# jacklishufan/InstructAny2Pix

Hardware: AMD Instinct MI355X
Metric: denoise-steps/sec (512x512, 50-step DDIM, batch 8) (higher is better)
Workload: dtype f16; 1 GPU; BASELINE configs[2]: 512x512, latent [8,4,64,64], 50-step DDIM, ctx 81 (77 text + 4 IP tokens), SDXL-base UNet + IP-Adapter; global_batch=8, parallelism=dp1, context_kv=projected in every step (reference schedule, as rounds 1-4), ranks=1, dist_backend=none (single process), weight_broadcast_route=none

## Files before the change

### instructany2pix_amd/csrc/attention_core.h

```cpp
#pragma once
#include "common.h"

#define MASKED (-1.0e30f)
#ifndef IA2P_ATTN_DMA
#define IA2P_ATTN_DMA 1
#endif
#ifndef IA2P_ATTN_PK
#define IA2P_ATTN_PK 1
#endif

__device__ __forceinline__ fp16x4 lds_tr16(const char* p) {
  return __builtin_amdgcn_ds_read_tr16_b64_v4f16((fp16x4 __attribute__((address_space(3)))*)p);
}

template <int NT>
__device__ __forceinline__ void stage_kv(const half_t* Kb, const half_t* Vb, int ld, int s0, int nsk, int tid, char* sK, char* sV) {
  typedef unsigned int u4 __attribute__((ext_vector_type(4)));
  u4 kreg[2 * NT], vreg[2 * NT];
#pragma unroll
  for (int u = 0; u < 2 * NT; ++u) {
    const int c = tid + 256 * u, row = c >> 3, pos = c & 7;
    const size_t off = (size_t)(s0 + min(row, nsk - 1)) * ld + pos * 8;
    kreg[u] = *(const u4*)(Kb + off);
    vreg[u] = *(const u4*)(Vb + off);
// ... 38 lines not shown
    if (write) {
      *(u4*)(sK + lrow * 128 + ((pos ^ ((lrow >> 1) & 7)) << 4)) = kreg[u] & keep;
      *(u4*)(sV + lrow * 128 + ((pos ^ (((lrow >> 1) & 1) << 2)) << 4)) = vreg[u] & keep;
    }
  }
}

typedef unsigned int attn_u4 __attribute__((ext_vector_type(4)));
constexpr int ATTN_PRE_TILES = 3;
struct AttnKvRegs { attn_u4 k[2 * ATTN_PRE_TILES], v[2 * ATTN_PRE_TILES]; };
__device__ __host__ __forceinline__ bool attn_kv_resident(const AttnArgs& p) {
  return ((p.seg[0].nkeys + 63) >> 6) + (p.nseg == 2 ? (p.seg[1].nkeys + 63) >> 6 : 0) <= ATTN_PRE_TILES;
}
__device__ __forceinline__ void attn_kv_load(const AttnArgs& p, int b, int hd, int tid, AttnKvRegs& rg) {
  typedef unsigned int u4 __attribute__((ext_vector_type(4)));
  const int nt0 = (p.seg[0].nkeys + 63) >> 6;
  const bool two = p.nseg == 2;
  const AttnSeg sg1 = two ? p.seg[1] : p.seg[0];
  const half_t* K0 = p.seg[0].K + (size_t)b * p.seg[0].rows_per_batch * p.seg[0].ld + hd * 64;
  const half_t* V0 = p.seg[0].V + (size_t)b * p.seg[0].rows_per_batch * p.seg[0].ld + hd * 64;
  const half_t* K1 = sg1.K + (size_t)b * sg1.rows_per_batch * sg1.ld + hd * 64;
  const half_t* V1 = sg1.V + (size_t)b * sg1.rows_per_batch * sg1.ld + hd * 64;
#pragma unroll
  for (int u = 0; u < 2 * ATTN_PRE_TILES; ++u) {
    const bool s1 = (u >> 1) >= nt0;
    const int c = tid + 256 * u, row = (c >> 3) - (s1 ? nt0 * 64 : 0), pos = c & 7;
    const size_t off = (size_t)min(row, (s1 ? sg1.nkeys : p.seg[0].nkeys) - 1) * (s1 ? sg1.ld : p.seg[0].ld) + pos * 8;
    rg.k[u] = *(const u4*)((s1 ? K1 : K0) + off);
    rg.v[u] = *(const u4*)((s1 ? V1 : V0) + off);
  }
}
template <bool FOLD = false>
__device__ __forceinline__ void attn_kv_store(const AttnArgs& p, int tid, const AttnKvRegs& rg, char* sK, char* sV) {
  typedef unsigned int u4 __attribute__((ext_vector_type(4)));
  const int n0 = p.seg[0].nkeys, n1 = p.nseg == 2 ? p.seg[1].nkeys : 0;
  const int nt0 = (n0 + 63) >> 6, nt = nt0 + ((n1 + 63) >> 6);
  const bool fold = FOLD && !(p.xcd_map & 4) && n1 > 0 && attn_fold_ok(n0, n1);
#pragma unroll
  for (int u = 0; u < 2 * ATTN_PRE_TILES; ++u) {
    if ((u >> 1) >= nt || (fold && u > 2 * nt0)) break;
    const bool s1 = (u >> 1) >= nt0;
    const int c = tid + 256 * u, pos = c & 7;
    int lrow = c >> 3;
    const int row = lrow - (s1 ? nt0 * 64 : 0);
    const unsigned keep = row < (s1 ? n1 : n0) ? 0xFFFFFFFFu : 0u;
    bool write = true;
    if (fold) {
      if (s1) { write = row < n1; lrow = n0 + row; }
      else write = lrow < n0 || lrow >= n0 + n1;
    }
    if (write) {
      *(u4*)(sK + lrow * 128 + ((pos ^ ((lrow >> 1) & 7)) << 4)) = rg.k[u] & keep;
      *(u4*)(sV + lrow * 128 + ((pos ^ (((lrow >> 1) & 1) << 2)) << 4)) = rg.v[u] & keep;
    }
  }
}

template <int MODE, bool PRE = false>
__device__ __forceinline__ void attn_core(const AttnArgs& p, int b, int hd, const h8 (&qf)[4], char* sK, char* sV, int tid, f16v (&otot)[2]) {
  const int lane = tid & 63;
  const int r31 = lane & 31, hh = lane >> 5;
  (void)r31;
  f16v o[2];
  float mrun = MASKED, lrun = 0.f;
#pragma unroll
  for (int d = 0; d < 2; ++d)
#pragma unroll
    for (int r = 0; r < 16; ++r) { o[d][r] = 0.f; if (MODE == 2) otot[d][r] = 0.f; }

  const int nt0 = (p.seg[0].nkeys + 63) >> 6, nt1 = p.nseg == 2 ? (p.seg[1].nkeys + 63) >> 6 : 0;
  const bool resident = PRE || (MODE != 0 && nt0 + nt1 <= 4);
  const int n0 = p.seg[0].nkeys, n1 = p.nseg == 2 ? p.seg[1].nkeys : 0;
  const bool fold = MODE == 1 && resident && !(p.xcd_map & 4) && attn_fold_ok(n0, n1);
  if (resident && !PRE) {
    const half_t* K0 = p.seg[0].K + (size_t)b * p.seg[0].rows_per_batch * p.seg[0].ld + hd * 64;
    const half_t* V0 = p.seg[0].V + (size_t)b * p.seg[0].rows_per_batch * p.seg[0].ld + hd * 64;
    const half_t* K1 = p.seg[1].K + (size_t)b * p.seg[1].rows_per_batch * p.seg[1].ld + hd * 64;
    const half_t* V1 = p.seg[1].V + (size_t)b * p.seg[1].rows_per_batch * p.seg[1].ld + hd * 64;
    switch (nt0 + nt1) {
      case 2: stage_kv2<2>(K0, V0, p.seg[0].ld, p.seg[0].nkeys, K1, V1, p.seg[1].ld, p.seg[1].nkeys, nt0, tid, sK, sV, fold); break;
      case 3: stage_kv2<3>(K0, V0, p.seg[0].ld, p.seg[0].nkeys, K1, V1, p.seg[1].ld, p.seg[1].nkeys, nt0, tid, sK, sV, fold); break;
      default: stage_kv2<4>(K0, V0, p.seg[0].ld, p.seg[0].nkeys, K1, V1, p.seg[1].ld, p.seg[1].nkeys, nt0, tid, sK, sV, fold); break;
    }
    __syncthreads();
  }
  float lt = 1.f;
  constexpr int NSEG = MODE == 0 ? 1 : 2;
#pragma unroll 1
  for (int sg = 0; sg < NSEG; ++sg) {
    if (MODE == 1 && fold && sg == 1) break;
    AttnSeg seg = sg == 0 ? p.seg[0] : p.seg[1];
    if (sg == 1 && p.w1_b) seg.weight = p.w1_b[b];
    const half_t* Kb = seg.K + (size_t)b * seg.rows_per_batch * seg.ld + hd * 64;
    const half_t* Vb = seg.V + (size_t)b * seg.rows_per_batch * seg.ld + hd * 64;
    const bool ip_tile = MODE == 1 && sg == 1;
    if (MODE == 2 || ip_tile) { mrun = MASKED; lrun = 0.f; }
    if (MODE == 2) {
#pragma unroll
      for (int d = 0; d < 2; ++d)
#pragma unroll
        for (int r = 0; r < 16; ++r) o[d][r] = 0.f;
    }

    constexpr bool DMA = IA2P_ATTN_DMA && MODE == 0 && !PRE;
    constexpr int SSZ = DMA ? 128 : 256;
    auto stage_dma = [&](int s0n, int buf) {
// ... 267 lines not shown
```

### instructany2pix_amd/csrc/gemm_epilogue.h

```cpp
#pragma once
#include "gemm_tile.h"
#include "gn_fold.h"

template <int BM, int BN, int NSTAGE, int WGM, int BK, int PP, int WGN, int XA, int HALO>
__device__ __forceinline__ void tile_epilogue(f4 (&acc)[BM / WGM / 16][BN / WGN / 16], const TileCtx& tc, const GemmArgs& p, const AttnArgs* xa, AttnKvRegs& kvr) {
  constexpr int NWAVE = WGM * WGN;
  constexpr int WM = BM / WGM, WN = BN / WGN;
  constexpr int MR = WM / 16, NR = WN / 16;
  constexpr int MRH = MR / 2;
  extern __shared__ __attribute__((aligned(1024))) char smem[];
  const int tid = threadIdx.x;
  const int lane = tid & 63;
  const int wave = __builtin_amdgcn_readfirstlane(tid >> 6);
  const int hM = tc.hM, hN = tc.hN, hK = tc.hK, tm = tc.tm, tn = tc.tn, bm0 = tc.bm0, bn0 = tc.bn0, tiles_m = tc.tiles_m, tiles_n = tc.tiles_n, split = tc.split, nsplit = tc.nsplit;
  const float ln_s1 = tc.ln_s1, ln_s2 = tc.ln_s2;
  (void)tiles_m; (void)hK;
  auto row_m = [&](int r) { return HALO ? tc.h_m0 + (r >> 4) * p.Wo + (r & 15) : bm0 + r; };
  auto frag_row = [](int i) constexpr { return PP == 2 ? (i / (MR / 2)) * (BM / 2) + (i % (MR / 2)) * 16 : i * 16; };
  auto frag_col = [](int j) constexpr { return PP == 2 ? (j / (NR / 2)) * (BN / 2) + (j % (NR / 2)) * 16 : j * 16; };
  const int wm0 = (wave / WGN) * (PP == 2 ? WM / 2 : WM), wn0 = (wave % WGN) * (PP == 2 ? WN / 2 : WN);
  const int frow = lane & 15, fq = lane >> 4;
  using EC = EpiCfg<BM, BN, NSTAGE, WGM, BK, WGN, PP>;
  constexpr int PITCH = EC::PITCH;
  constexpr int NT = NWAVE * 64, CR = EC::CR;
  float* tile = (float*)smem;
  const bool reg_epi = XA == 0 && EC::REG_EPI && nsplit == 1 && p.vec8 != 0 && (hN & 7) == 0 && !p.act;
  char* cbase = smem + (reg_epi ? EC::T16_BYTES : EC::TILE_BYTES);
  float* ln_rows = (float*)cbase;
  float* ln_cs = ln_rows + 2 * BM;
  float* ln_lb = ln_cs + BN;
  int* sk_flag = (int*)(ln_lb + BN);
  float2* part = (float2*)(ln_lb + BN + 4);
  const float2* phi = (const float2*)(cbase + (reg_epi ? EC::EXTRA16 - EC::LUT_BYTES : EC::extra_nolut(CR)));
  __syncthreads();
  if (p.ln_stats) {
    if (tid < BM) {
      const float2 mr = ln_mean_rstd_f(ln_s1, ln_s2, hK, p.ln_eps);
      ln_rows[tid] = mr.x;
      ln_rows[BM + tid] = mr.y;
    }
    if constexpr (XA == 4) {
      if (tid < BN / 4) {
        const int n = ((tid * 4) >> 6) * (hN / 3) + tn * 64 + ((tid * 4) & 63);
        *(f4*)(ln_cs + tid * 4) = *(const f4*)(p.ln_cs + n);
        *(f4*)(ln_lb + tid * 4) = *(const f4*)(p.ln_bias + n);
      }
    } else if (tid < BN / 4 && bn0 + tid * 4 < hN) {
      *(f4*)(ln_cs + tid * 4) = *(const f4*)(p.ln_cs + bn0 + tid * 4);
      *(f4*)(ln_lb + tid * 4) = *(const f4*)(p.ln_bias + bn0 + tid * 4);
    }
  }
  unsigned pfacc = 0, pfv[8] = {0, 0, 0, 0, 0, 0, 0, 0};
  if ((PP == 1 || PP == 2) && p.pf) {
    const long nwg = (long)tiles_m * tiles_n * nsplit;
    const long per = ((p.pf_bytes + nwg - 1) / nwg + 255) & ~255L;
    const long lo = (long)blockIdx.x * per, hi = min(lo + per, p.pf_bytes & ~15L);
    const char* src = (const char*)p.pf;
    constexpr long SW = NWAVE * 64 * 16;
    if (lo < hi)
      for (long o = lo + tid * 16; o < hi; o += 8 * SW) {
#pragma unroll
        for (int u = 0; u < 8; ++u) pfacc ^= pfv[u];
#pragma unroll
        for (int u = 0; u < 8; ++u) pfv[u] = *(const unsigned*)(src + min(o + u * SW, hi - 16));
#ifdef IA2P_PP_EAGER_PF
#pragma unroll
        for (int u = 0; u < 8; ++u) asm volatile("" : "+v"(pfv[u]));
#endif
      }
  }
  auto pf_sink = [&]() {
    if (PP == 1 || PP == 2) asm volatile("" ::"v"(pfacc), "v"(pfv[0]), "v"(pfv[1]), "v"(pfv[2]), "v"(pfv[3]), "v"(pfv[4]), "v"(pfv[5]), "v"(pfv[6]), "v"(pfv[7]));
  };
  const float e_as = p.acc_scale == 0.f ? 1.f : p.acc_scale, e_bs = p.bias_scale == 0.f ? 1.f : p.bias_scale;
  const bool fast = p.vec8 != 0 && (hN & 7) == 0;
  const __amdgpu_buffer_rsrc_t c_rsrc = wt_rsrc((void*)p.C, (size_t)hM * p.ldc * 2);
  auto store_c8 = [&](size_t elem, h8 o) {
    if (p.c_wt) store16_wt(c_rsrc, elem * 2, o);
    else *(h8*)(p.C + elem) = o;
  };
  auto tl = [&](int r, int c) -> f4 { return *(const f4*)(tile + (size_t)r * PITCH + ((c ^ (r & 7)) << 2)); };
  auto acc_to_tile = [&](int ch) {
    if constexpr (PP == 2) {
      static_assert(PP != 2 || (EC::NCHUNK == 2 && CR == BM / 2), "8-phase tile: one epilogue chunk per row half");
      auto half = [&](auto h_tag) {
        constexpr int H = decltype(h_tag)::value;
// ... 20 lines not shown
        }
      }
    }
  };
  if constexpr (XA == 4) {
    static_assert(XA != 4 || (BM == 256 && BN == 192 && WGM == 4 && WGN == 2 && (PP == 0 || PP == 3)), "fused QKV + self-attention: 256 x 192 tiles, 8 waves");
    char* sK = smem;
    char* sV = smem + 32768;
    char* sQ = smem + 65536;
    __syncthreads();
#pragma unroll
    for (int i = 0; i < MR; ++i) {
      const int r = wm0 + i * 16 + frow;
      const float mu = p.ln_stats ? ln_rows[r] : 0.f, rs = p.ln_stats ? ln_rows[BM + r] : 1.f;
#pragma unroll
      for (int j = 0; j < NR; ++j) {
        const int cl = wn0 + j * 16 + fq * 4;
        float v[4] = {acc[i][j][0], acc[i][j][1], acc[i][j][2], acc[i][j][3]};
        if (p.ln_stats) {
#pragma unroll
          for (int e = 0; e < 4; ++e) v[e] = ln_fold_f(v[e], mu, rs, ln_cs[cl + e], ln_lb[cl + e]);
        } else if (p.bias) {
          const h4 hb = *(const h4*)(p.bias + (cl >> 6) * (hN / 3) + tn * 64 + (cl & 63));
#pragma unroll
          for (int e = 0; e < 4; ++e) v[e] += (float)hb[e];
        }
        h4 o;
#pragma unroll
        for (int e = 0; e < 4; ++e) o[e] = (half_t)v[e];
        const int which = cl >> 6, d = cl & 63, chunk = d >> 3, sub = (d & 7) * 2;
        const int sw = which == 0 ? (r & 7) : which == 1 ? ((r >> 1) & 7) : (((r >> 1) & 1) << 2);
        char* img = which == 0 ? sQ : which == 1 ? sK : sV;
        *(h4*)(img + r * 128 + ((chunk ^ sw) << 4) + sub) = o;
      }
    }
    __syncthreads();
    IA2P_STAMP(if (tid == 0 && p.partial) ((unsigned long long*)p.partial)[8 * blockIdx.x + 7] = __builtin_amdgcn_s_memrealtime();)
    const int r31 = lane & 31, hh = lane >> 5;
    h8 qf[4];
    {
      const int r = wave * 32 + r31;
#pragma unroll
      for (int s = 0; s < 4; ++s) qf[s] = *(const h8*)(sQ + r * 128 + (((2 * s + hh) ^ (r & 7)) << 4));
    }
    const AttnArgs& ap = *xa;
    f16v otot[2];
    attn_core<0, true>(ap, tm, tn, qf, sK, sV, tid, otot);
    IA2P_STAMP(if (tid == 0 && p.partial) ((unsigned long long*)p.partial)[8 * blockIdx.x + 6] = __builtin_amdgcn_s_memrealtime();)
    attn_store_o(otot, ap.O, (size_t)ap.B * ap.Nq * ap.ldo, tm, wave * 32, tn, ap.Nq, ap.ldo, sQ + wave * 4096, lane, (ap.xcd_map & 2) != 0);
    IA2P_STAMP(
      asm volatile("s_waitcnt vmcnt(0)" ::: "memory");
      __syncthreads();
      if (tid == 0 && p.partial) ((unsigned long long*)p.partial)[8 * blockIdx.x + 5] = __builtin_amdgcn_s_memrealtime();
    )
    return;
  } else if constexpr (XA != 0) {
    static_assert(BM == 128 && BN == 64 && WGM == 2 && WGN == 2 && !PP && EC::NCHUNK == 1, "fused cross-attention: 128 x 64 tiles, 4 waves");
    IA2P_STAMP(unsigned long long* xo = p.partial ? (unsigned long long*)p.partial + 8 * blockIdx.x : nullptr;)
    acc_to_tile(0);
    __syncthreads();
    const int r31 = lane & 31, hh = lane >> 5;
    h8 qf[4];
    {
      const int r = wave * 32 + r31;
      const float mu = p.ln_stats ? ln_rows[r] : 0.f, rs = p.ln_stats ? ln_rows[BM + r] : 1.f;
#pragma unroll
      for (int s = 0; s < 4; ++s) {
        const int cl = 16 * s + 8 * hh;
        const f4 x0 = tl(r, cl >> 2), x1 = tl(r, (cl >> 2) + 1);
        float v[8] = {x0[0], x0[1], x0[2], x0[3], x1[0], x1[1], x1[2], x1[3]};
        if (p.ln_stats) {
#pragma unroll
          for (int e = 0; e < 8; ++e) v[e] = ln_fold_f(v[e], mu, rs, ln_cs[cl + e], ln_lb[cl + e]);
        } else {
#pragma unroll
          for (int e = 0; e < 8; ++e) v[e] *= e_as;
          if (p.bias) {
            const h8 hb = *(const h8*)(p.bias + bn0 + cl);
#pragma unroll
            for (int e = 0; e < 8; ++e) v[e] = fmaf((float)hb[e], e_bs, v[e]);
          }
        }
#pragma unroll
        for (int e = 0; e < 8; ++e) qf[s][e] = (half_t)v[e];
      }
    }
    __syncthreads();
    const AttnArgs& ap = *xa;
    const int b = bm0 / ap.Nq, q0 = bm0 - b * ap.Nq + wave * 32, hd = tn;
    f16v otot[2];
    attn_kv_store<XA - 1 == 1>(ap, tid, kvr, smem, smem + 32768);
    __syncthreads();
    IA2P_STAMP(if (tid == 0 && xo) xo[6] = __builtin_amdgcn_s_memrealtime();)
    attn_core<XA - 1, true>(ap, b, hd, qf, smem, smem + 32768, tid, otot);
    __syncthreads();
    IA2P_STAMP(if (tid == 0 && xo) xo[7] = __builtin_amdgcn_s_memrealtime();)
    attn_store_o(otot, ap.O, (size_t)ap.B * ap.Nq * ap.ldo, b, q0, hd, ap.Nq, ap.ldo, smem + wave * 4096, lane, (ap.xcd_map & 2) != 0);
  IA2P_STAMP(
    asm volatile("s_waitcnt vmcnt(0)" ::: "memory");
    __syncthreads();
    if (tid == 0 && xo) xo[5] = __builtin_amdgcn_s_memrealtime();
  )
    return;
  }
  if constexpr (XA == 0 && EC::REG_EPI) {
  if (reg_epi) {
// ... 542 lines not shown
```

### instructany2pix_amd/csrc/gemm_kernel.h

```cpp
#pragma once
#include "gemm_epilogue.h"

template <int BM, int BN, int NSTAGE, bool CONV, int WGM = 2, int BK = 64, int PP = 0, int WGN = 2, int XA = 0, bool SUB = false>
__device__ __forceinline__ void gemm_tile_body(const half_t* hA, const half_t* hW, const half_t* hzero, int hM, int hN, int hK, int hlda, int hldw, int hrpb, int hbstride,
                                               int hroff, int hsplitk, int hgroup_w, int hflags, const GemmArgs& p, const AttnArgs* xa, const float* pre_ln_stats = nullptr, int pre_ln_slots = 0, int bid0 = 0) {
  static_assert(PP != 1 || (WGM * WGN == 8 && (WGM == 4 || WGM == 8) && NSTAGE == 3), "ping-pong schedule: 8 waves (two groups of 4 by tile rows), 3-stage ring");
  static_assert(PP != 3 || (WGM == 4 && NSTAGE == 2 && !CONV), "two-slot ping-pong schedule: 8 waves, 2 k-tile slots");
  static_assert(PP != 2 || (WGM == 2 && WGN == 4 && NSTAGE == 2 && BK == 64 && BM == 256 && (BN == 256 || BN == 128) && XA == 0), "8-phase schedule: 256-row tiles, 2 x 4 waves, two k-tile buffers");
  constexpr int NWAVE = WGM * WGN;
  constexpr int WM = BM / WGM, WN = BN / WGN;
  constexpr int MR = WM / 16, NR = WN / 16;
  constexpr int ROWB = 2 * BK, CPR = ROWB / 16, RPP = 1024 / ROWB;
  using BS = BStage<BN, BK, NWAVE, PP>;
  constexpr int A_PW = BM / RPP / NWAVE, B_PW = BS::HI;
  constexpr bool B_UNEVEN = BS::UNEVEN;
  constexpr int BNL = BS::BNL;
  static_assert(BM % (RPP * NWAVE) == 0 && BN % 16 == 0 && WN % 16 == 0 && WM % 16 == 0, "tile / wave layout");
  constexpr int STAGE = (BM + BNL) * ROWB;
  constexpr int KSUB = BK / 32;
  extern __shared__ __attribute__((aligned(1024))) char smem[];

  int tid_ = threadIdx.x;
  if constexpr (SUB) asm volatile("" : "+v"(tid_));
  const int tid = tid_;
// ... 463 lines not shown
    };
    zero_acc();
    if (nk > 1) wait_vm_barrier<HLPS>(); else wait_vm_barrier<0>();
    if (wave >= NWAVE / 2) bar2();
    auto ktile = [&](int t, auto slot_tag) {
      constexpr int SL = decltype(slot_tag)::value;
      rd_b(SL, H0{}, wf0);
      __builtin_amdgcn_sched_barrier(0);
      rd_a(SL, H0{});
      __builtin_amdgcn_sched_barrier(0);
      if (t + 1 < nk) stage_part(SL ^ 1, S_A1{});
      __builtin_amdgcn_sched_barrier(0);
      asm volatile("s_waitcnt lgkmcnt(%0)" ::"n"(KSUB * MRH) : "memory");
      bar1();
      mmq(H0{}, H0{}, wf0);
      bar2();
      rd_b(SL, H1{}, wf1);
      __builtin_amdgcn_sched_barrier(0);
      if (t + 2 < nk) stage_part(SL, S_B0{});
      bar1();
      conv_prepare();
      mmq(H0{}, H1{}, wf1);
      bar2();
      rd_a(SL, H1{});
      __builtin_amdgcn_sched_barrier(0);
      if (t + 2 < nk) stage_part(SL, S_A0{});
      bar1();
      mmq(H1{}, H1{}, wf1);
      bar2();
      if (t + 2 < nk) {
        stage_part(SL, S_B1{});
        __builtin_amdgcn_sched_barrier(0);
        asm volatile("s_waitcnt vmcnt(%0)" ::"n"(HLPS) : "memory");
      } else {
        __builtin_amdgcn_sched_barrier(0);
        asm volatile("s_waitcnt vmcnt(0)" ::: "memory");
      }
      bar1();
      mmq(H1{}, H0{}, wf0);
      bar2();
    };
    for (int t = 0; t < nk; t += 2) {
      ktile(t, std::integral_constant<int, 0>{});
      if (t + 1 < nk) ktile(t + 1, std::integral_constant<int, 1>{});
    }
    if (wave < NWAVE / 2) bar2();
  } else {
  int cur = 0, nxt = NSTAGE - 1;
  for (int kt = 0; kt < nk; ++kt) {
    const int ahead = nk - 1 - kt;
    wait_ring<NSTAGE - 2, LPS>(ahead < NSTAGE - 2 ? ahead : NSTAGE - 2);
    IA2P_STAMP(if (IA2P_STAMP_AT == 4 && kt == 0) stamp_put(p, nsplit, 7);)
    if (kt + NSTAGE - 1 < nk) stage(kt + NSTAGE - 1, nxt);
    if constexpr (XA != 0 && XA != 4) {
      if (kt == 0) attn_kv_load(*xa, bm0 / xa->Nq, tn, tid, kvr);
    }
    const char* base = smem + cur * STAGE;
    if constexpr (MR * NR <= 16) {
      h8 af[KSUB][MR], wf[KSUB][NR];
#pragma unroll
      for (int kk = 0; kk < KSUB; ++kk) {
        const int coff = ((kk * 4 + fq) ^ fswz) << 4;
#pragma unroll
        for (int i = 0; i < MR; ++i) af[kk][i] = *(const h8*)(base + a_off + i * 16 * ROWB + coff);
#pragma unroll
        for (int j = 0; j < NR; ++j) wf[kk][j] = *(const h8*)(base + w_off + j * 16 * ROWB + coff);
      }
      __builtin_amdgcn_sched_barrier(0);
      conv_prepare();
#pragma unroll
      for (int kk = 0; kk < KSUB; ++kk)
#pragma unroll
        for (int i = 0; i < MR; ++i)
#pragma unroll
          for (int j = 0; j < NR; ++j)
            acc[i][j] = __builtin_amdgcn_mfma_f32_16x16x32_f16(wf[kk][j], af[kk][i], acc[i][j], 0, 0, 0);
    } else {
#pragma unroll
      for (int kk = 0; kk < KSUB; ++kk) {
        const int coff = ((kk * 4 + fq) ^ fswz) << 4;
        h8 af[MR], wf[NR];
#pragma unroll
        for (int i = 0; i < MR; ++i) af[i] = *(const h8*)(base + a_off + i * 16 * ROWB + coff);
#pragma unroll
        for (int j = 0; j < NR; ++j) wf[j] = *(const h8*)(base + w_off + j * 16 * ROWB + coff);
        if (kk == 0) conv_prepare();
#pragma unroll
        for (int i = 0; i < MR; ++i)
#pragma unroll
          for (int j = 0; j < NR; ++j)
            acc[i][j] = __builtin_amdgcn_mfma_f32_16x16x32_f16(wf[j], af[i], acc[i][j], 0, 0, 0);
      }
    }
    cur = cur + 1 == NSTAGE ? 0 : cur + 1;
    nxt = nxt + 1 == NSTAGE ? 0 : nxt + 1;
  }

  }
  TileCtx tc;
  tc.hM = hM; tc.hN = hN; tc.hK = hK; tc.tm = tm; tc.tn = tn; tc.bm0 = bm0; tc.bn0 = bn0; tc.tiles_m = tiles_m; tc.tiles_n = tiles_n; tc.split = split; tc.nsplit = nsplit;
  tc.h_m0 = 0; tc.ln_s1 = ln_s1; tc.ln_s2 = ln_s2;
  IA2P_STAMP(
    if (tid == 0 && stamp_base(p, nsplit)) {
      unsigned long long* o = stamp_base(p, nsplit) + 8 * blockIdx.x;
      const unsigned long long r1 = __builtin_amdgcn_s_memrealtime();
      o[0] = __builtin_amdgcn_s_memtime() - stamp_c0; o[1] = r1 - stamp_r0; o[2] = stamp_entry; o[3] = stamp_r0; o[4] = r1;
    }
// ... 42 lines not shown
```

### instructany2pix_amd/csrc/gemm_tile.h

```cpp
#pragma once
#include "common.h"
#include "attention_core.h"

#include <algorithm>
#include <cmath>
#include <cstdint>
#include <cstdlib>
#include <type_traits>

bool ia2p_splitk_inkernel(int M, int N, int splitk);
int ia2p_gemm_variant_ran(const GemmArgs& a, bool conv, int v);
int ia2p_sk_counter_capacity();
int* ia2p_sk_counters(hipStream_t s, int tiles);
void ia2p_sk_counters_invalidate();
const float* ia2p_phi_lut();

#ifndef IA2P_LIN_BUF
#define IA2P_LIN_BUF 1
#endif
#define BLDS16(rsrc, ldsptr, voff, soff) \
  __builtin_amdgcn_raw_ptr_buffer_load_lds(rsrc, (__attribute__((address_space(3))) void*)(ldsptr), 16, voff, soff, 0, 0)
#define GLDS16(gptr, ldsptr)                                                                         \
  __builtin_amdgcn_global_load_lds((const __attribute__((address_space(1))) void*)(gptr),            \
                                   (__attribute__((address_space(3))) void*)(ldsptr), 16, 0, 0)

template <int N> __device__ __forceinline__ void wait_vm_barrier() {
  asm volatile("s_waitcnt vmcnt(%0)\n\ts_barrier" ::"n"(N) : "memory");
}

template <int MAXT, int LPS> __device__ __forceinline__ void wait_ring(int tiles) {
  static_assert(MAXT * LPS <= 63, "vmcnt immediate");
  if constexpr (MAXT <= 0) wait_vm_barrier<0>();
  else {
    if (tiles >= MAXT) wait_vm_barrier<MAXT * LPS>();
    else wait_ring<MAXT - 1, LPS>(tiles);
  }
}

template <int BK> __device__ __forceinline__ int lds_swz(int row) { return BK == 64 ? (row >> 1) & 7 : (-(row >> 2)) & 3; }


template <int BN, int BK, int NWAVE, int PP>
struct BStage {
  static constexpr int RPP = 1024 / (2 * BK), P = BN / RPP, HI = (P + NWAVE - 1) / NWAVE;
  static constexpr bool UNEVEN = PP != 0 && P % NWAVE != 0 && P == (NWAVE / 2) * (2 * HI - 1);
  static constexpr int BNL = UNEVEN ? BN : HI * NWAVE * RPP;
};

template <int BM, int BN, int NSTAGE, int WGM, int BK, int WGN = 2, int PP = 0>
struct EpiCfg {
  static constexpr int BNL = BStage<BN, BK, WGM * WGN, PP>::BNL;
  static constexpr int STAGE_BYTES = NSTAGE * (BM + BNL) * 2 * BK;
  static constexpr int PITCH = ((BN / 4 + 7) & ~7) * 4;
  static constexpr bool POW2 = ((BN / 8) & (BN / 8 - 1)) == 0;
  static constexpr int LUT_BYTES = BN % 32 == 0 ? ((IA2P_PHI_LUT_N * 8 + 15) & ~15) : 0;
  static constexpr int extra_nolut(int cr) { return (2 * BM + 2 * BN + 4) * 4 + (POW2 ? 0 : cr * (BN / 8) * 8); }
  static constexpr int extra(int cr) { return extra_nolut(cr) + LUT_BYTES; }
  static constexpr int LIMIT = (PP == 2 || (BM == 256 && BN == 192)) ? 160 * 1024 : STAGE_BYTES > 80 * 1024 ? STAGE_BYTES : 80 * 1024;
  static constexpr int NCHUNK = (PP != 2 && BM * PITCH * 4 + extra(BM) <= LIMIT) ? 1 : 2;
  static_assert(WGM % NCHUNK == 0, "a chunk holds whole wave rows");
  static constexpr int CR = BM / NCHUNK;
  static constexpr int TILE_BYTES = CR * PITCH * 4;
  static_assert(TILE_BYTES + extra(CR) <= LIMIT, "epilogue staging does not fit");
  static constexpr int SMEM_F32 = STAGE_BYTES > TILE_BYTES + extra(CR) ? STAGE_BYTES : TILE_BYTES + extra(CR);
  static constexpr int P16 = BN * 2 + 16, T16_BYTES = BM * P16;
  static constexpr int EXTRA16 = (2 * BM + 2 * BN + 4) * 4 + (POW2 ? 0 : BM * (BN / 8) * 8) + LUT_BYTES;
#ifndef IA2P_REG_EPI_MIN
#define IA2P_REG_EPI_MIN 4097
#endif
  static constexpr bool REG_EPI = T16_BYTES + EXTRA16 <= LIMIT && BM * BN >= IA2P_REG_EPI_MIN;
  static constexpr int SMEM = REG_EPI && T16_BYTES + EXTRA16 > SMEM_F32 ? T16_BYTES + EXTRA16 : SMEM_F32;
};

#ifdef IA2P_CLOCK_STAMP
#define IA2P_STAMP(...) __VA_ARGS__
#ifndef IA2P_STAMP_AT
#define IA2P_STAMP_AT 0
#endif
__device__ __forceinline__ unsigned long long* stamp_base(const GemmArgs& p, int nsplit) {
  return p.stamp ? p.stamp : (nsplit == 1 ? (unsigned long long*)p.partial : nullptr);
}
__device__ __forceinline__ void stamp_put(const GemmArgs& p, int nsplit, int slot) {
  unsigned long long* b = stamp_base(p, nsplit);
  if (threadIdx.x == 0 && b) b[8 * blockIdx.x + slot] = __builtin_amdgcn_s_memrealtime();
}
#else
#define IA2P_STAMP(...)
#endif

__device__ __forceinline__ int udiv_small(int a, int b) {
  int q = (int)((float)a * __builtin_amdgcn_rcpf((float)b));
  const int r = a - q * b;
  q += (r >= b ? 1 : 0) - (r < 0 ? 1 : 0);
  return q;
}
__device__ __forceinline__ void tile_order(int bid, int tiles_m, int tiles_n, int group_w, int m_fastest, int& tm, int& tn) {
  {
    const int nwg = tiles_m * tiles_n;
    const int q = nwg >> 3, r = nwg & 7, x = bid & 7, i = bid >> 3;
    bid = (x < r ? x * (q + 1) : r * (q + 1) + (x - r) * q) + i;
// ... 61 lines not shown
```

### instructany2pix_amd/csrc/qxattn.hip

```cpp
#include "gemm_kernel.h"
#include "launch_args.h"

#include <cstring>

#ifndef IA2P_QX_STAGES
#define IA2P_QX_STAGES 2
#endif
template <int MODE>
__global__ __launch_bounds__(256, 2) void qproj_xattn_kernel(const half_t* hA, const half_t* hW, const half_t* hzero, const float* h_ln_stats, int hM, int hN, int hK, int hlda, int hldw,
                                                             int h_slots_gw, const GemmArgs p, const AttnArgs xa) {
  gemm_tile_body<128, 64, IA2P_QX_STAGES, false, 2, 64, 0, 2, MODE + 1>(hA, hW, hzero, hM, hN, hK, hlda, hldw, 0, 0, 0, 0, IA2P_SKGW_GW(h_slots_gw), IA2P_SKGW_FLAGS(h_slots_gw), p, &xa, h_ln_stats,
                                                                        IA2P_SKGW_LO8(h_slots_gw));
}

bool ia2p_qproj_xattn_ok(const GemmArgs& a, const AttnArgs& x) {
  return x.Nq > 0 && x.Nq % 128 == 0 && a.M == x.B * x.Nq && a.N == x.heads * 64 && a.K >= 64 && a.K % 64 == 0 && a.splitk <= 1 && !a.rpb && !a.geglu && !a.residual && !a.rowvec &&
         !a.stats_out && !a.act && x.nseg >= 1 && x.nseg <= 2 && x.seg[0].nkeys > 0 && (x.nseg == 1 || x.seg[1].nkeys > 0) &&
         (!a.bias || ((((uintptr_t)a.bias) & 15) == 0 && a.N % 8 == 0)) && x.ldo % 8 == 0 && ((((uintptr_t)x.O) & 15) == 0) &&
         ia2p_fits_buffer(a.rpb ? ((size_t)a.M / a.rpb + 1) * (size_t)(a.bstride > 0 ? a.bstride : 0) + a.roff + a.rpb : (size_t)a.M, a.lda) && ia2p_fits_buffer(a.N, a.ldw) &&
         attn_kv_resident(x);
}

hipError_t ia2p_launch_qproj_xattn(const GemmArgs& a, const AttnArgs& x, hipStream_t s) {
  if (!ia2p_qproj_xattn_ok(a, x)) return hipErrorInvalidValue;
  constexpr int BM = 128, BN = 64, SMEM = EpiCfg<128, 64, IA2P_QX_STAGES, 2, 64, 2>::SMEM > 65536 ? EpiCfg<128, 64, IA2P_QX_STAGES, 2, 64, 2>::SMEM : 65536;
  static_assert(EpiCfg<BM, BN, IA2P_QX_STAGES, 2, 64, 2>::SMEM <= SMEM, "LDS budget");
  static bool attr_set[64] = {false};
  int dev = 0;
  (void)hipGetDevice(&dev);
  if (dev < 0 || dev >= 64 || !attr_set[dev]) {
    hipError_t e = hipFuncSetAttribute((const void*)qproj_xattn_kernel<0>, hipFuncAttributeMaxDynamicSharedMemorySize, SMEM);
    if (e == hipSuccess) e = hipFuncSetAttribute((const void*)qproj_xattn_kernel<1>, hipFuncAttributeMaxDynamicSharedMemorySize, SMEM);
    if (e == hipSuccess) e = hipFuncSetAttribute((const void*)qproj_xattn_kernel<2>, hipFuncAttributeMaxDynamicSharedMemorySize, SMEM);
    if (e != hipSuccess) return e;
    if (dev >= 0 && dev < 64) attr_set[dev] = true;
  }
  const int tiles_n = a.N / BN, tiles = (a.M / BM) * tiles_n;
  GemmArgs b = a;
  b.vec8 = 1; b.splitk = 0; b.sk_counters = nullptr;
#ifndef IA2P_CLOCK_STAMP
  b.partial = nullptr;
#endif
  b.group_w = ia2p_tile_group_w(tiles, tiles_n, SMEM, BM, BN);
  AttnArgs y = x;
  y.xcd_map = (((ia2p_wt_mask() & 8) && (size_t)x.B * x.Nq * x.ldo * 2 < (size_t)0x7ffffff0) ? 2 : 0) | (ia2p_attn_fold_enabled() ? 0 : 4);
  const int extra = (a.pf && a.pf_bytes >= 4096) ? a.pf_blocks : 0;
  int slots_gw;
  if (tiles + extra >= (1 << 21) || !ia2p_pack_skgw(b.ln_stats ? b.ln_slots : 0, b.group_w, b.m_fastest, b.ln_stats != nullptr, &slots_gw)) return hipErrorInvalidValue;
  const int mode = y.nseg == 1 ? 0 : (y.seg[1].nkeys <= 64 && y.seg[0].weight != 0.f) ? 1 : 2;
#define IA2P_QX_LAUNCH(MODE)                                                                                                                   \
  hipLaunchKernelGGL(qproj_xattn_kernel<MODE>, dim3(tiles + extra), dim3(256), SMEM, s, b.A, b.W, b.zero, b.ln_stats, b.M, b.N, b.K, b.lda, b.ldw, slots_gw, b, y)
  if (mode == 0) IA2P_QX_LAUNCH(0);
  else if (mode == 1) IA2P_QX_LAUNCH(1);
  else IA2P_QX_LAUNCH(2);
#undef IA2P_QX_LAUNCH
  return hipGetLastError();
}


__global__ __launch_bounds__(512, 2) void qkv_sattn_kernel(const half_t* hA, const half_t* hW, const half_t* hzero, const float* h_ln_stats, int hM, int hN, int hK, int hlda, int hldw,
                                                           int h_slots_gw, const GemmArgs p, const AttnArgs xa, const CtxKvArgs ck) {
#ifndef IA2P_SATTN_PP
#define IA2P_SATTN_PP 3
#endif
  gemm_tile_body<256, 192, 2, false, 4, 64, IA2P_SATTN_PP, 2, 4>(hA, hW, hzero, hM, hN, hK, hlda, hldw, 0, 0, 0, 0, IA2P_SKGW_GW(h_slots_gw), IA2P_SKGW_FLAGS(h_slots_gw), p, &xa, h_ln_stats, IA2P_SKGW_LO8(h_slots_gw));
}

bool ia2p_qkv_sattn_ok(const GemmArgs& a, const AttnArgs& x) {
  return x.Nq == 256 && x.B > 0 && a.M == x.B * 256 && a.N == 3 * x.heads * 64 && a.K >= 64 && a.K % 64 == 0 && a.splitk <= 1 && !a.geglu && !a.residual && !a.rowvec &&
         !a.stats_out && !a.act && !a.rpb && x.nseg == 1 && x.ldo % 8 == 0 && ((((uintptr_t)x.O) & 15) == 0) && (!a.bias || ((((uintptr_t)a.bias) & 7) == 0)) &&
         (!a.ln_stats || (((((uintptr_t)a.ln_cs) | ((uintptr_t)a.ln_bias)) & 15) == 0)) && ia2p_fits_buffer(a.M, a.lda) && ia2p_fits_buffer(a.N, a.ldw);
}

constexpr int CK_BM = 128, CK_BN = 160;
int ia2p_cu_count() {
  static int cus[64] = {0};
  int dev = 0;
  if (hipGetDevice(&dev) != hipSuccess || dev < 0 || dev >= 64) { (void)hipGetLastError(); return 0; }
  if (!cus[dev]) {
    int n = 0;
    if (hipDeviceGetAttribute(&n, hipDeviceAttributeMultiprocessorCount, dev) != hipSuccess) { (void)hipGetLastError(); n = 0; }
    cus[dev] = n > 0 ? n : -1;
  }
  return cus[dev] > 0 ? cus[dev] : 0;
}
int ia2p_qkv_sattn_ctx_tiles(const CtxKvSlice& k) {
  const int tn = (k.N + CK_BN - 1) / CK_BN;
  return ((k.B * k.Lt + CK_BM - 1) / CK_BM) * tn + (k.Li > 0 ? ((k.B * k.Li + CK_BM - 1) / CK_BM) * tn : 0);
}
bool ia2p_qkv_sattn_ctx_ok(const AttnArgs& x, const CtxKvSlice& k) {
  if (k.B < 1 || k.B != x.B || k.Lt < 1 || k.Li < 0 || k.L != k.Lt + k.Li || k.N < 8 || k.N % 8 || k.K < 64 || k.K % 64 || k.lda < k.K || k.ldc < k.N) return false;
  if (k.Lt > 0xffff || k.Li > 0xffff || (long)k.B * k.L >= (1L << 21)) return false;
  if (!ia2p_fits_buffer((size_t)k.B * k.L + k.L, k.lda) || !ia2p_fits_buffer(k.N, k.K)) return false;
  return (long)x.B * x.heads + ia2p_qkv_sattn_ctx_tiles(k) <= ia2p_cu_count();
}

hipError_t ia2p_launch_qkv_sattn(const GemmArgs& a, const AttnArgs& x, hipStream_t s, const CtxKvSlice* ctx) {
  if (!ia2p_qkv_sattn_ok(a, x)) return hipErrorInvalidValue;
  constexpr int SMEM = EpiCfg<256, 192, 2, 4, 64, 2, 0>::SMEM;
  static_assert(SMEM >= 96 * 1024 + (2 * 256 + 2 * 192) * 4, "K / V / Q images + row and column constants");
  constexpr int CK_SMEM = EpiCfg<CK_BM, CK_BN, 3, 4, 64, 2, 1>::SMEM;
  static_assert(CK_SMEM <= SMEM, "a context K/V tile runs in the fused tile's LDS request");
  CtxKvArgs ck;
  memset(&ck, 0, sizeof ck);
// ... 41 lines not shown
```

Baseline: 56.08 steps/s.

## Stage cross-attention K/V into LDS via buffer_load_lds DMA in Q-projection kernel

Adds a new variant of the fused Q-projection + cross-attention kernel that loads the context K/V tiles straight into LDS with buffer_load_lds at the first k-step, instead of holding them in registers and writing them to LDS later. The epilogue writes the projected Q tile into LDS directly from the accumulators and runs attention on the DMA-staged K/V. This is meant to cut register pressure and the register-to-LDS copy while overlapping the K/V fetch with the GEMM main loop. The LDS footprint is sized so two workgroups still fit per CU. It only applies when the context fits in two 64-key tiles, which holds for 81 keys with folding.

```diff
diff --git a/instructany2pix_amd/csrc/attention_core.h b/instructany2pix_amd/csrc/attention_core.h
--- a/instructany2pix_amd/csrc/attention_core.h
+++ b/instructany2pix_amd/csrc/attention_core.h
@@ -114,6 +114,40 @@
     if (write) {
       *(u4*)(sK + lrow * 128 + ((pos ^ ((lrow >> 1) & 7)) << 4)) = rg.k[u] & keep;
       *(u4*)(sV + lrow * 128 + ((pos ^ (((lrow >> 1) & 1) << 2)) << 4)) = rg.v[u] & keep;
+    }
+  }
+}
+
+constexpr int ATTN_DMA_TILES = 2;
+__device__ __host__ __forceinline__ bool attn_kv_dma_ok(const AttnArgs& p, bool may_fold) {
+  const int n0 = p.seg[0].nkeys, n1 = p.nseg == 2 ? p.seg[1].nkeys : 0;
+  const bool fold = may_fold && !(p.xcd_map & 4) && n1 > 0 && attn_fold_ok(n0, n1);
+  if ((long)n0 * p.seg[0].ld >= (1L << 29) || (n1 > 0 && (long)n1 * p.seg[1].ld >= (1L << 29))) return false;
+  return ((n0 + 63) >> 6) + (fold ? 0 : (n1 + 63) >> 6) <= ATTN_DMA_TILES;
+}
+template <bool FOLD>
+__device__ __forceinline__ void attn_kv_dma(const AttnArgs& p, int b, int hd, int wave, int lane, char* sK, char* sV) {
+  const int n0 = p.seg[0].nkeys, n1 = p.nseg == 2 ? p.seg[1].nkeys : 0;
+  const bool fold = FOLD && !(p.xcd_map & 4) && n1 > 0 && attn_fold_ok(n0, n1);
+  const int r1 = fold ? n0 : ((n0 + 63) >> 6) * 64;
+  const bool isV = wave >= 2;
+  const int ld0 = p.seg[0].ld, ld1 = p.seg[1].ld;
+  const half_t* b0 = (isV ? p.seg[0].V : p.seg[0].K) + (size_t)b * p.seg[0].rows_per_batch * ld0 + hd * 64;
+  const half_t* b1 = b0;
+  if (n1 > 0) b1 = (isV ? p.seg[1].V : p.seg[1].K) + (size_t)b * p.seg[1].rows_per_batch * ld1 + hd * 64;
+  const __amdgpu_buffer_rsrc_t rs0 = __builtin_amdgcn_make_buffer_rsrc((void*)b0, 0, ((n0 - 1) * ld0 + 64) * 2, 0x00020000);
+  const __amdgpu_buffer_rsrc_t rs1 = __builtin_amdgcn_make_buffer_rsrc((void*)b1, 0, n1 > 0 ? ((n1 - 1) * ld1 + 64) * 2 : 0, 0x00020000);
+  char* img = isV ? sV : sK;
+#pragma unroll
+  for (int u = 0; u < 4 * ATTN_DMA_TILES; ++u) {
+    const int pi = (wave & 1) * (4 * ATTN_DMA_TILES) + u;
+    const int row = pi * 8 + (lane >> 3), cp = lane & 7;
+    const int g = cp ^ (isV ? (((row >> 1) & 1) << 2) : ((row >> 1) & 7));
+    const bool in1 = row >= r1 && row < r1 + n1;
+    char* dst = img + pi * 1024;
+    if (!in1) __builtin_amdgcn_raw_ptr_buffer_load_lds(rs0, (__attribute__((address_space(3))) void*)dst, 16, row < n0 ? (row * ld0 + g * 8) * 2 : 0x7fffff00, 0, 0, 0);
+    if (pi * 8 + 8 > r1 && pi * 8 < r1 + n1) {
+      if (in1) __builtin_amdgcn_raw_ptr_buffer_load_lds(rs1, (__attribute__((address_space(3))) void*)dst, 16, ((row - r1) * ld1 + g * 8) * 2, 0, 0, 0);
     }
   }
 }
diff --git a/instructany2pix_amd/csrc/gemm_epilogue.h b/instructany2pix_amd/csrc/gemm_epilogue.h
--- a/instructany2pix_amd/csrc/gemm_epilogue.h
+++ b/instructany2pix_amd/csrc/gemm_epilogue.h
@@ -32,6 +32,7 @@
   int* sk_flag = (int*)(ln_lb + BN);
   float2* part = (float2*)(ln_lb + BN + 4);
   const float2* phi = (const float2*)(cbase + (reg_epi ? EC::EXTRA16 - EC::LUT_BYTES : EC::extra_nolut(CR)));
+  if constexpr (xa_kv_dma(XA)) asm volatile("s_waitcnt vmcnt(0)" ::: "memory");
   __syncthreads();
   if (p.ln_stats) {
     if (tid < BM) {
@@ -158,6 +159,60 @@
       asm volatile("s_waitcnt vmcnt(0)" ::: "memory");
       __syncthreads();
       if (tid == 0 && p.partial) ((unsigned long long*)p.partial)[8 * blockIdx.x + 5] = __builtin_amdgcn_s_memrealtime();
+    )
+    return;
+  } else if constexpr (xa_kv_dma(XA)) {
+    static_assert(BM == 128 && BN == 64 && WGM == 2 && WGN == 2 && !PP, "fused cross-attention: 128 x 64 tiles, 4 waves");
+    IA2P_STAMP(unsigned long long* xo = p.partial ? (unsigned long long*)p.partial + 8 * blockIdx.x : nullptr;)
+    char* sQ = smem;
+    char* sK = smem + QX_RING_BYTES(NSTAGE);
+    char* sV = sK + ATTN_DMA_TILES * 8192;
+    __syncthreads();
+#pragma unroll
+    for (int i = 0; i < MR; ++i) {
+      const int r = wm0 + i * 16 + frow;
+      const float mu = p.ln_stats ? ln_rows[r] : 0.f, rs = p.ln_stats ? ln_rows[BM + r] : 1.f;
+#pragma unroll
+      for (int j = 0; j < NR; ++j) {
+        const int cl = wn0 + j * 16 + fq * 4;
+        float v[4] = {acc[i][j][0], acc[i][j][1], acc[i][j][2], acc[i][j][3]};
+        if (p.ln_stats) {
+#pragma unroll
+          for (int e = 0; e < 4; ++e) v[e] = ln_fold_f(v[e], mu, rs, ln_cs[cl + e], ln_lb[cl + e]);
+        } else {
+#pragma unroll
+          for (int e = 0; e < 4; ++e) v[e] *= e_as;
+          if (p.bias) {
+            const h4 hb = *(const h4*)(p.bias + bn0 + cl);
+#pragma unroll
+            for (int e = 0; e < 4; ++e) v[e] = fmaf((float)hb[e], e_bs, v[e]);
+          }
+        }
+        h4 o;
+#pragma unroll
+        for (int e = 0; e < 4; ++e) o[e] = (half_t)v[e];
+        *(h4*)(sQ + r * 128 + (((cl >> 3) ^ (r & 7)) << 4) + (cl & 7) * 2) = o;
+      }
+    }
+    __syncthreads();
+    const int r31 = lane & 31, hh = lane >> 5;
+    h8 qf[4];
+    {
+      const int r = wave * 32 + r31;
+#pragma unroll
+      for (int s = 0; s < 4; ++s) qf[s] = *(const h8*)(sQ + r * 128 + (((2 * s + hh) ^ (r & 7)) << 4));
+    }
+    IA2P_STAMP(if (tid == 0 && xo) xo[6] = __builtin_amdgcn_s_memrealtime();)
+    const AttnArgs& ap = *xa;
+    const int b = bm0 / ap.Nq, q0 = bm0 - b * ap.Nq + wave * 32, hd = tn;
+    f16v otot[2];
+    attn_core<xa_mode(XA), true>(ap, b, hd, qf, sK, sV, tid, otot);
+    IA2P_STAMP(if (tid == 0 && xo) xo[7] = __builtin_amdgcn_s_memrealtime();)
+    attn_store_o(otot, ap.O, (size_t)ap.B * ap.Nq * ap.ldo, b, q0, hd, ap.Nq, ap.ldo, sQ + wave * 4096, lane, (ap.xcd_map & 2) != 0);
+    IA2P_STAMP(
+      asm volatile("s_waitcnt vmcnt(0)" ::: "memory");
+      __syncthreads();
+      if (tid == 0 && xo) xo[5] = __builtin_amdgcn_s_memrealtime();
     )
     return;
   } else if constexpr (XA != 0) {
diff --git a/instructany2pix_amd/csrc/gemm_kernel.h b/instructany2pix_amd/csrc/gemm_kernel.h
--- a/instructany2pix_amd/csrc/gemm_kernel.h
+++ b/instructany2pix_amd/csrc/gemm_kernel.h
@@ -539,7 +539,9 @@
     wait_ring<NSTAGE - 2, LPS>(ahead < NSTAGE - 2 ? ahead : NSTAGE - 2);
     IA2P_STAMP(if (IA2P_STAMP_AT == 4 && kt == 0) stamp_put(p, nsplit, 7);)
     if (kt + NSTAGE - 1 < nk) stage(kt + NSTAGE - 1, nxt);
-    if constexpr (XA != 0 && XA != 4) {
+    if constexpr (xa_kv_dma(XA)) {
+      if (kt == 0) attn_kv_dma<xa_mode(XA) == 1>(*xa, bm0 / xa->Nq, tn, wave, lane, smem + QX_RING_BYTES(NSTAGE), smem + QX_RING_BYTES(NSTAGE) + ATTN_DMA_TILES * 8192);
+    } else if constexpr (xa_cross(XA)) {
       if (kt == 0) attn_kv_load(*xa, bm0 / xa->Nq, tn, tid, kvr);
     }
     const char* base = smem + cur * STAGE;
diff --git a/instructany2pix_amd/csrc/gemm_tile.h b/instructany2pix_amd/csrc/gemm_tile.h
--- a/instructany2pix_amd/csrc/gemm_tile.h
+++ b/instructany2pix_amd/csrc/gemm_tile.h
@@ -46,6 +46,11 @@
   static constexpr bool UNEVEN = PP != 0 && P % NWAVE != 0 && P == (NWAVE / 2) * (2 * HI - 1);
   static constexpr int BNL = UNEVEN ? BN : HI * NWAVE * RPP;
 };
+
+constexpr bool xa_cross(int xa) { return xa != 0 && xa != 4; }
+constexpr bool xa_kv_dma(int xa) { return xa > 4; }
+constexpr int xa_mode(int xa) { return xa > 4 ? xa - 5 : xa - 1; }
+constexpr int QX_RING_BYTES(int nstage) { return nstage * (128 + 64) * 128; }
 
 template <int BM, int BN, int NSTAGE, int WGM, int BK, int WGN = 2, int PP = 0>
 struct EpiCfg {
diff --git a/instructany2pix_amd/csrc/qxattn.hip b/instructany2pix_amd/csrc/qxattn.hip
--- a/instructany2pix_amd/csrc/qxattn.hip
+++ b/instructany2pix_amd/csrc/qxattn.hip
@@ -6,10 +6,10 @@
 #ifndef IA2P_QX_STAGES
 #define IA2P_QX_STAGES 2
 #endif
-template <int MODE>
+template <int MODE, bool KVD>
 __global__ __launch_bounds__(256, 2) void qproj_xattn_kernel(const half_t* hA, const half_t* hW, const half_t* hzero, const float* h_ln_stats, int hM, int hN, int hK, int hlda, int hldw,
                                                              int h_slots_gw, const GemmArgs p, const AttnArgs xa) {
-  gemm_tile_body<128, 64, IA2P_QX_STAGES, false, 2, 64, 0, 2, MODE + 1>(hA, hW, hzero, hM, hN, hK, hlda, hldw, 0, 0, 0, 0, IA2P_SKGW_GW(h_slots_gw), IA2P_SKGW_FLAGS(h_slots_gw), p, &xa, h_ln_stats,
+  gemm_tile_body<128, 64, IA2P_QX_STAGES, false, 2, 64, 0, 2, MODE + (KVD ? 5 : 1)>(hA, hW, hzero, hM, hN, hK, hlda, hldw, 0, 0, 0, 0, IA2P_SKGW_GW(h_slots_gw), IA2P_SKGW_FLAGS(h_slots_gw), p, &xa, h_ln_stats,
                                                                         IA2P_SKGW_LO8(h_slots_gw));
 }
 
@@ -23,15 +23,20 @@
 
 hipError_t ia2p_launch_qproj_xattn(const GemmArgs& a, const AttnArgs& x, hipStream_t s) {
   if (!ia2p_qproj_xattn_ok(a, x)) return hipErrorInvalidValue;
-  constexpr int BM = 128, BN = 64, SMEM = EpiCfg<128, 64, IA2P_QX_STAGES, 2, 64, 2>::SMEM > 65536 ? EpiCfg<128, 64, IA2P_QX_STAGES, 2, 64, 2>::SMEM : 65536;
-  static_assert(EpiCfg<BM, BN, IA2P_QX_STAGES, 2, 64, 2>::SMEM <= SMEM, "LDS budget");
+  constexpr int BM = 128, BN = 64, SMEM_REG = EpiCfg<128, 64, IA2P_QX_STAGES, 2, 64, 2>::SMEM > 65536 ? EpiCfg<128, 64, IA2P_QX_STAGES, 2, 64, 2>::SMEM : 65536;
+  constexpr int SMEM_DMA = QX_RING_BYTES(IA2P_QX_STAGES) + 2 * ATTN_DMA_TILES * 8192;
+  static_assert(EpiCfg<BM, BN, IA2P_QX_STAGES, 2, 64, 2>::SMEM <= SMEM_REG && EpiCfg<BM, BN, IA2P_QX_STAGES, 2, 64, 2>::SMEM_F32 <= QX_RING_BYTES(IA2P_QX_STAGES), "LDS budget");
+  static_assert(IA2P_QX_STAGES != 2 || SMEM_DMA == 80 * 1024, "two workgroups per CU");
   static bool attr_set[64] = {false};
   int dev = 0;
   (void)hipGetDevice(&dev);
   if (dev < 0 || dev >= 64 || !attr_set[dev]) {
-    hipError_t e = hipFuncSetAttribute((const void*)qproj_xattn_kernel<0>, hipFuncAttributeMaxDynamicSharedMemorySize, SMEM);
-    if (e == hipSuccess) e = hipFuncSetAttribute((const void*)qproj_xattn_kernel<1>, hipFuncAttributeMaxDynamicSharedMemorySize, SMEM);
-    if (e == hipSuccess) e = hipFuncSetAttribute((const void*)qproj_xattn_kernel<2>, hipFuncAttributeMaxDynamicSharedMemorySize, SMEM);
+    hipError_t e = hipFuncSetAttribute((const void*)qproj_xattn_kernel<0, false>, hipFuncAttributeMaxDynamicSharedMemorySize, SMEM_REG);
+    if (e == hipSuccess) e = hipFuncSetAttribute((const void*)qproj_xattn_kernel<1, false>, hipFuncAttributeMaxDynamicSharedMemorySize, SMEM_REG);
+    if (e == hipSuccess) e = hipFuncSetAttribute((const void*)qproj_xattn_kernel<2, false>, hipFuncAttributeMaxDynamicSharedMemorySize, SMEM_REG);
+    if (e == hipSuccess) e = hipFuncSetAttribute((const void*)qproj_xattn_kernel<0, true>, hipFuncAttributeMaxDynamicSharedMemorySize, SMEM_DMA);
+    if (e == hipSuccess) e = hipFuncSetAttribute((const void*)qproj_xattn_kernel<1, true>, hipFuncAttributeMaxDynamicSharedMemorySize, SMEM_DMA);
+    if (e == hipSuccess) e = hipFuncSetAttribute((const void*)qproj_xattn_kernel<2, true>, hipFuncAttributeMaxDynamicSharedMemorySize, SMEM_DMA);
     if (e != hipSuccess) return e;
     if (dev >= 0 && dev < 64) attr_set[dev] = true;
   }
@@ -41,15 +46,22 @@
 #ifndef IA2P_CLOCK_STAMP
   b.partial = nullptr;
 #endif
-  b.group_w = ia2p_tile_group_w(tiles, tiles_n, SMEM, BM, BN);
+  b.group_w = ia2p_tile_group_w(tiles, tiles_n, SMEM_REG, BM, BN);
   AttnArgs y = x;
   y.xcd_map = (((ia2p_wt_mask() & 8) && (size_t)x.B * x.Nq * x.ldo * 2 < (size_t)0x7ffffff0) ? 2 : 0) | (ia2p_attn_fold_enabled() ? 0 : 4);
   const int extra = (a.pf && a.pf_bytes >= 4096) ? a.pf_blocks : 0;
   int slots_gw;
   if (tiles + extra >= (1 << 21) || !ia2p_pack_skgw(b.ln_stats ? b.ln_slots : 0, b.group_w, b.m_fastest, b.ln_stats != nullptr, &slots_gw)) return hipErrorInvalidValue;
   const int mode = y.nseg == 1 ? 0 : (y.seg[1].nkeys <= 64 && y.seg[0].weight != 0.f) ? 1 : 2;
-#define IA2P_QX_LAUNCH(MODE)                                                                                                                   \
-  hipLaunchKernelGGL(qproj_xattn_kernel<MODE>, dim3(tiles + extra), dim3(256), SMEM, s, b.A, b.W, b.zero, b.ln_stats, b.M, b.N, b.K, b.lda, b.ldw, slots_gw, b, y)
+#ifndef IA2P_QX_KV_DMA
+#define IA2P_QX_KV_DMA 1
+#endif
+  const bool kvd = IA2P_QX_KV_DMA && attn_kv_dma_ok(y, mode == 1);
+#define IA2P_QX_LAUNCH(MODE)                                                                                                                                                    \
+  do {                                                                                                                                                                          \
+    if (kvd) hipLaunchKernelGGL((qproj_xattn_kernel<MODE, true>), dim3(tiles + extra), dim3(256), SMEM_DMA, s, b.A, b.W, b.zero, b.ln_stats, b.M, b.N, b.K, b.lda, b.ldw, slots_gw, b, y);   \
+    else hipLaunchKernelGGL((qproj_xattn_kernel<MODE, false>), dim3(tiles + extra), dim3(256), SMEM_REG, s, b.A, b.W, b.zero, b.ln_stats, b.M, b.N, b.K, b.lda, b.ldw, slots_gw, b, y);     \
+  } while (0)
   if (mode == 0) IA2P_QX_LAUNCH(0);
   else if (mode == 1) IA2P_QX_LAUNCH(1);
   else IA2P_QX_LAUNCH(2);
```

Result: no change. 56.28 steps/s (median of 6 runs) (+0.3%).
